# RoboSafe-Lab/Controllable-Latent-Diffusion-for-Traffic-Simulation

Measured on AMD Instinct MI355X. Metric: denoising-step·agent/s, higher is better.
Workload: dtype f32; 1 GPU; BASELINE configs[2]: 32 scenes x 64 agents per GPU, 100 denoising steps (DDPM ancestral loop of the reference), latent seq 52 x 4, cond 256, CFG w=2.0 (2 U-Net passes per step, non_cond_feat); target-speed guidance gradient through decoder + roll-out on every step t > 0; + LSTM decode + unicycle roll-out; scenes_total=32, agents_this_rank=2048, agents_total=2048, denoise_steps=100, guidance_gradient=True, sim_steps_per_bench_step=0, weights=random init (synth seed 0)

## Files before the change

controllable-latent-diffusion-for-traffic-simulation_amd/_lib.py:

```python
from __future__ import annotations

import ctypes as C
import os

PKG_DIR = os.path.dirname(os.path.abspath(__file__))
LIB_PATH = os.environ.get("CLD_LIB_PATH") or os.path.join(PKG_DIR, "libcld_hip.so")


class CldError(RuntimeError):
    pass


class CldConfig(C.Structure):
    _fields_ = [
        ("horizon", C.c_int32), ("latent_dim", C.c_int32), ("cond_dim", C.c_int32), ("base_dim", C.c_int32),
        ("dim_mults", C.c_int32 * 3), ("hidden", C.c_int32), ("n_timesteps", C.c_int32),
        ("step_time", C.c_float), ("acce_bound", C.c_float * 2), ("v_bound", C.c_float * 2),
        ("max_steer", C.c_float), ("max_yawvel", C.c_float),
        ("norm_mean", C.c_float * 6), ("norm_std", C.c_float * 6),
        ("precision", C.c_int32),
    ]


PRECISIONS = {"f32": 0, "f16x2": 1}
OPTIMIZERS = {"adam": 0, "sgd": 1}
KERNELS = {"guide": 0, "decode": 1, "encode": 2, "unet": 3, "context": 4, "conv5": 5}
KERNEL_FORMS = {
    "guide": {"auto": 0, "valu": 1, "mfma": 2, "quad": 3},
    "decode": {"auto": 0, "valu": 1, "mfma": 2},
    "encode": {"auto": 0, "valu": 1, "mfma": 2},
    "unet": {"auto": 0, "layers": 1, "chain": 2, "chain1": 3, "chain4": 4, "chainw": 5, "chainw2": 6, "chainw1": 7},
    "context": {"auto": 0, "direct": 1, "winograd": 2, "winograd_f2": 3},
    "conv5": {"auto": 0, "direct": 1, "winograd": 2, "winograd_whole": 3, "winograd_ksplit": 4},
}
FORMS = {name: v for forms in KERNEL_FORMS.values() for name, v in forms.items()}


def form_id(kind: str, name: str) -> int:
    if kind not in KERNEL_FORMS:
        raise ValueError(f"unknown kernel '{kind}' (one of {sorted(KERNEL_FORMS)})")
# ... 74 lines not shown
                                     C.c_int32, _P]),
    "cld_agent_collision": (C.c_int, [_P, _P, C.POINTER(CldCollision), _P, _P, _P, C.c_int32, _P]),
    "cld_map_collision_loss": (C.c_int, [_P, _P, C.POINTER(CldMapCollision), _P, _P, _P, C.c_int32, _P]),
    "cld_goal_loss": (C.c_int, [_P, _P, C.POINTER(CldGoal), _P, _P, _P, C.c_int32, _P]),
    "cld_set_goal_term": (C.c_int, [_P, C.POINTER(CldGoal)]),
    "cld_world_step": (C.c_int, [_P, _P, _P, _P, C.c_int32, _P, _P, C.c_int32, _P]),
    "cld_profile_enable": (C.c_int, [_P, C.c_int32]),
    "cld_profile_read": (C.c_int, [_P, C.POINTER(C.c_double), C.POINTER(C.c_int64), C.POINTER(C.c_double)]),
    "cld_profile_read_executed": (C.c_int, [_P, C.POINTER(C.c_double), C.POINTER(C.c_double), C.POINTER(C.c_double), C.POINTER(C.c_int32)]),
    "cld_set_stride": (C.c_int, [_P, C.c_int32]),
    "cld_debug_lds_floor": (C.c_int, [_P, C.c_size_t]),
    "cld_debug_force_kernel": (C.c_int, [_P, C.c_int32, C.c_int32]),
    "cld_debug_conv5_form": (C.c_int, [C.c_int32, C.c_int32, C.c_int32, C.c_int32, C.c_int64, C.c_int32]),
    "cld_debug_conv5_items": (C.c_int, [C.c_int32, C.c_int32, C.c_int64, C.c_int32]),
    "cld_debug_unet_span": (C.c_int, [_P, C.c_int32, _P, _P, _P, C.c_int32, _P, _P, C.c_int32, _P, C.c_size_t, _P]),
    "cld_debug_context_layer": (C.c_int, [_P, C.c_int32, _P, _P, _P, C.c_int32, C.c_int32, _P]),
    "cld_debug_context_pass_size": (C.c_int, [C.c_int32]),
    "cld_debug_stamps": (C.c_int, [_P, _P, C.c_int32]),
    "cld_debug_guide_stamps": (C.c_int, [_P]),
    "cld_unet_param_count": (C.c_int, [_P]),
    "cld_unet_param_info": (C.c_int, [_P, C.c_int32, C.POINTER(C.c_char_p), C.POINTER(C.c_size_t), C.POINTER(C.c_size_t),
                                      C.POINTER(C.c_int32), C.POINTER(C.c_int32)]),
    "cld_unet_param_floats": (C.c_size_t, [_P]),
    "cld_unet_tape_bytes": (C.c_size_t, [_P, C.c_int32]),
    "cld_unet_train_workspace_bytes": (C.c_size_t, [_P, C.c_int32]),
    "cld_unet_train_forward": (C.c_int, [_P, _P, _P, _P, _P, _P, _P, C.c_size_t, C.c_int32, _P, C.c_size_t, _P]),
    "cld_unet_backward": (C.c_int, [_P, _P, _P, _P, _P, _P, C.c_size_t, _P, _P, _P, _P, C.c_int32, C.c_int32, _P, C.c_size_t, _P]),
    "cld_vae_param_count": (C.c_int, [_P]),
    "cld_vae_param_info": (C.c_int, [_P, C.c_int32, C.POINTER(C.c_char_p), C.POINTER(C.c_size_t), C.POINTER(C.c_size_t),
                                     C.POINTER(C.c_int32), C.POINTER(C.c_int32)]),
# ... 36 lines not shown
```

controllable-latent-diffusion-for-traffic-simulation_amd/csrc/cld_api.hip:

```cpp
#include <hip/hip_runtime.h>

#include <cmath>
#include <cstdio>
#include <cstdlib>
#include <cstring>
#include <map>
#include <string>
#include <vector>

#include "../../include/cld.h"
#include "cld_kernels.h"
#include "train.h"

using namespace cld;

namespace {

constexpr int T = 52, D = 4, COND = 256, TE = 32, NCB = 1792, ACT = 3328;
constexpr int NBUF = 8;

struct ConvLayer {
    ConvGeom g{};
    bool has_a = false, has_b = false;
    float *wfrag = nullptr, *bias = nullptr, *gamma = nullptr, *beta = nullptr;
    float* ufrag_edge = nullptr;
    float* ufrag = nullptr;
    bool wino_launch = false;
    int c_out = 0, c1_real = 0, c1_pad = 0, c2 = 0, ly = 0, off0 = 0, orow0 = 0;
    int cb_off = -1;
};

struct ResBlock { ConvLayer c0, c1, res; bool has_res = false; };
constexpr long kProfStride = 10;
constexpr int kChainSmall = 944;
const char* const kResnet = "context_encoder.map_encoder.encoder_heads.map_model.";

}

struct cld_handle_s {
    cld_config cfg{};
    int stride = 1;
    int precision = CLD_PRECISION_F32;
// ... 21 lines not shown
    bool has_context = false;
    float *stem_w = nullptr, *stem_scale = nullptr, *stem_shift = nullptr;
    Conv2dLayer rn_conv[4][2][2], rn_ds[4];
    ContextHeadArgs ctx_head{};
    DynParams dyn{};
    bool prof_on = false;
    std::vector<hipEvent_t> prof_ev;
    size_t prof_used = 0;
    double prof_flop = 0.0;
    double prof_exec_flop = 0.0;
    double eval_alg_flop = 0.0, eval_exec_flop = 0.0;
    int eval_launches = 0;
    unsigned long long* stamp_buf = nullptr;
    int stamp_layer = -1, launch_counter = 0;
    size_t lds_floor = 0;
    long eval_counter = 0;
};

namespace {

int fail(cld_handle h, int code, const std::string& msg) {
    if (h) h->err = msg;
    return code;
}
#define HIPCK(h, expr)                                                                           \
    do {                                                                                         \
        hipError_t e__ = (expr);                                                                 \
        if (e__ != hipSuccess)                                                                   \
            return fail(h, CLD_ERR_HIP, std::string(#expr) + ": " + hipGetErrorString(e__));     \
    } while (0)
// ... 96 lines not shown
                        out[o++] = wget(16 * nt + (lane & 15), 16 * kgg + 4 * (lane >> 4) + s, t);
    return out;
}

template <class F>
std::vector<float> pack_latent_conv_weights(F&& wget, int c_out) {
    const int ntn = c_out / 16;
    std::vector<float> out((size_t)ntn * 64 * 8, 0.f);
    for (int nt = 0; nt < ntn; ++nt)
        for (int lane = 0; lane < 64; ++lane) {
            float* o = &out[((size_t)nt * 64 + lane) * 8];
            const int co = 16 * nt + (lane & 15), kk = lane >> 4;
            for (int s = 0; s < 4; ++s) o[s] = wget(co, s, kk);
            o[4] = wget(co, kk, 4);
        }
    return out;
}

constexpr float kWScale = 64.0f;
template <class F>
std::vector<float> pack_conv_weights_split(F&& wget, int c_out, int cin_virtual, int ntaps) {
    const int nchunk = cin_virtual / 32, ntn = c_out / 16;
    std::vector<_Float16> out((size_t)nchunk * ntaps * ntn * 1024);
    size_t o = 0;
    for (int c = 0; c < nchunk; ++c)
        for (int t = 0; t < ntaps; ++t)
            for (int nt = 0; nt < ntn; ++nt) {
                for (int plane = 0; plane < 2; ++plane)
                    for (int lane = 0; lane < 64; ++lane)
                        for (int j = 0; j < 8; ++j) {
// ... 128 lines not shown
    return conv5_takes_winograd(l.g.l_in, l.c1_real, l.c2, l.c_out, b_pad, h->force_kernel[CLD_KERNEL_CONV5]);
}
void count_flop(cld_handle h, const ConvLayer& l, int b_pad, double* alg, double* exec) {
    const double cin = (double)(l.c1_real + l.c2);
    *alg = 2.0 * (double)b_pad * l.g.lm * (l.g.ntaps * cin) * l.c_out;
    if (use_wino1d(h, l, b_pad)) *exec = 2.0 * (double)wino1d_row_planes(l.g.l_in, l.c_out, b_pad, wino_item_form(h)) * cin * l.c_out;
    else *exec = 2.0 * (double)b_pad * l.g.lm * (l.g.padc ? 20.0 : (double)(l.g.ntaps * (l.c1_pad + l.c2))) * l.c_out;
}
void count_launch(cld_handle h, const ConvLayer& l, int b_pad) {
    double alg, exec;
    count_flop(h, l, b_pad, &alg, &exec);
    h->eval_alg_flop += alg;
    h->eval_exec_flop += exec;
    h->eval_launches++;
}
hipError_t launch_one(cld_handle h, const ConvLayer& l, const ConvGeom& g, const ConvArgs& a, int b_pad, hipStream_t s) {
    count_launch(h, l, b_pad);
    if (use_wino1d(h, l, b_pad)) {
        ConvArgs w = a;
        w.wfrag = l.ufrag;
        w.wfrag_edge = l.ufrag_edge;
        return launch_wino1d(w, l.g.l_in, b_pad, wino_item_form(h), s);
    }
    return launch_conv(g, a, b_pad, s);
}
hipError_t launch_maybe_timed(cld_handle h, const ConvLayer& l, const ConvGeom& g, const ConvArgs& a, int b_pad, hipStream_t s) {
    const bool timed = h->prof_on && g.l_in == 13 && g.ntaps == 5 && g.epi == EPI_GN_MISH && l.c_out == 256 && l.c1_real == 256 &&
                       (h->eval_counter % kProfStride) == 0;
    if (!timed) return launch_one(h, l, g, a, b_pad, s);
    if (h->prof_used + 2 > h->prof_ev.size()) {
        for (int i = 0; i < 2; ++i) {
            hipEvent_t ev;
            hipError_t e = hipEventCreate(&ev);
            if (e != hipSuccess) return e;
            h->prof_ev.push_back(ev);
        }
    }
    hipError_t e = hipEventRecord(h->prof_ev[h->prof_used], s);
    if (e != hipSuccess) return e;
    e = launch_one(h, l, g, a, b_pad, s);
    if (e != hipSuccess) return e;
    e = hipEventRecord(h->prof_ev[h->prof_used + 1], s);
    h->prof_used += 2;
    double alg, exec;
    count_flop(h, l, b_pad, &alg, &exec);
    h->prof_flop += alg;
    h->prof_exec_flop += exec;
    return e;
}

hipError_t run_pair(cld_handle h, const ConvLayer& la, const ConvArgs& aa, const ConvLayer& lb, const ConvArgs& ab,
                    int b_pad, hipStream_t s) {
    ConvGeom ga, gb;
    if (!pick_tiling(la, b_pad, &ga, 2) || !pick_tiling(lb, b_pad, &gb, 2)) return hipErrorInvalidValue;
#ifdef CLD_EXPERIMENTS
// ... 3 lines not shown
    h->launch_counter += 2;
    if (use_wino1d(h, la, b_pad) || use_wino1d(h, lb, b_pad)) {
        hipError_t e = launch_maybe_timed(h, la, ga, aa, b_pad, s);
        return e != hipSuccess ? e : launch_maybe_timed(h, lb, gb, ab, b_pad, s);
    }
    if (ga.nwn == gb.nwn && ga.ks == gb.ks && conv_pair_supported(ga, gb)) {
        count_launch(h, la, b_pad);
        count_launch(h, lb, b_pad);
        h->eval_launches--;
        return launch_conv_pair(ga, aa, gb, ab, b_pad, s);
    }
    hipError_t e = launch_maybe_timed(h, la, ga, aa, b_pad, s);
    return e != hipSuccess ? e : launch_maybe_timed(h, lb, gb, ab, b_pad, s);
}

hipError_t run_args(cld_handle h, const ConvLayer& l, ConvArgs a, int b_pad, hipStream_t s);
hipError_t run_conv(cld_handle h, const ConvLayer& l, const float* x1, const float* x2, float* y, const float* res,
                    const float* cb, const float* tb_row, int b_pad, hipStream_t s) {
    return run_args(h, l, make_args(h, l, x1, x2, y, res, cb, tb_row), b_pad, s);
}
hipError_t run_args(cld_handle h, const ConvLayer& l, ConvArgs a, int b_pad, hipStream_t s) {
#ifdef CLD_EXPERIMENTS
    static const int stop_after = getenv("CLD_DEBUG_STOP") ? atoi(getenv("CLD_DEBUG_STOP")) : 1 << 30;
    if (h->launch_counter >= stop_after) return hipSuccess;
#endif
    a.stamps = (h->stamp_buf && h->launch_counter == h->stamp_layer) ? h->stamp_buf : nullptr;
    h->launch_counter++;
    ConvGeom g;
    if (!pick_tiling(l, b_pad, &g)) return hipErrorInvalidValue;
    return launch_maybe_timed(h, l, g, a, b_pad, s);
}

bool use_chains(cld_handle h, int b_pad) {
    if (h->precision != CLD_PRECISION_F32) return false;
    const int f = h->force_kernel[CLD_KERNEL_UNET];
    if (f == CLD_FORM_LAYERS) return false;
    if (f == CLD_FORM_CHAIN || f == CLD_FORM_CHAIN_TILE1 || f == CLD_FORM_CHAIN_TILE4 || f == CLD_FORM_CHAIN_WINO || f == CLD_FORM_CHAIN_WINO2 || f == CLD_FORM_CHAIN_WINO1) return true;
    (void)b_pad;
    return true;
}
int chain_tile(cld_handle h, int b_pad) {
    const int f = h->force_kernel[CLD_KERNEL_UNET];
    if (f == CLD_FORM_CHAIN_TILE1) return 1;
    if (f == CLD_FORM_CHAIN_TILE4 || f == CLD_FORM_CHAIN_WINO) return 4;
    return b_pad <= kChainSmall ? 1 : 4;
// ... 13 lines not shown
}

constexpr int kSpans = 12;
constexpr int kSpanIn[kSpans] = {-1, 6, 2, 4, 6, 2, 5, 2, 3, 2, 6, 3};
constexpr int kSpanSkip[kSpans] = {-1, -1, -1, -1, -1, -1, -1, -1, 5, -1, -1, 4};
constexpr int kSpanOut[kSpans] = {6, 2, 4, 6, 2, 5, 2, 3, 2, 6, 3, 7};
constexpr int kSpanL[kSpans + 1] = {52, 26, 26, 26, 13, 13, 13, 13, 13, 13, 13, 26, 52};
constexpr int kSpanC[kSpans + 1] = {4, 64, 128, 128, 128, 256, 256, 256, 256, 128, 128, 128, 4};
hipError_t run_unet_span(cld_handle h, const Ws& w, const float* x, int t_idx, int b_pad, int span, hipStream_t s) {
    const float* tbr = t_idx >= 0 ? h->tb + (size_t)t_idx * NCB : nullptr;
    float* const* b = w.buf;
    hipError_t e;
#define RC(...) do { e = run_conv(h, __VA_ARGS__, w.cb, tbr, b_pad, s); if (e != hipSuccess) return e; } while (0)
    auto resblock = [&](const ResBlock& rb, const float* in1, const float* in2, float* out) -> hipError_t {
        const float* r = in1;
        if (rb.has_res) {
            e = run_pair(h, rb.c0, make_args(h, rb.c0, in1, in2, b[1], nullptr, w.cb, tbr),
                         rb.res, make_args(h, rb.res, in1, in2, b[0], nullptr, w.cb, tbr), b_pad, s);
            if (e != hipSuccess) return e;
            r = b[0];
        } else {
            RC(rb.c0, in1, in2, b[1], nullptr);
        }
        RC(rb.c1, b[1], nullptr, out, r);
        return hipSuccess;
    };
#define RB(...) do { e = resblock(__VA_ARGS__); if (e != hipSuccess) return e; } while (0)
    switch (span) {
    case 0:
    if (use_chains(h, b_pad)) {
// ... 190 lines not shown
    return CLD_OK;
}

int cld_debug_lds_floor(cld_handle h, size_t bytes) {
    if (!h) return CLD_ERR_ARG;
    h->lds_floor = bytes;
    return CLD_OK;
}

int cld_debug_force_kernel(cld_handle h, int32_t which, int32_t form) {
    if (!h || which < 0 || which > 5 || form < 0 || form > (which == CLD_KERNEL_GUIDE || which == CLD_KERNEL_CONTEXT ? 3 : which == CLD_KERNEL_CONV5 ? 4 : (which == CLD_KERNEL_UNET ? 7 : 2))) return fail(h, CLD_ERR_ARG, "cld_debug_force_kernel: bad argument");
    h->force_kernel[which] = form;
    return CLD_OK;
}

int cld_debug_conv5_form(int32_t l_in, int32_t c1, int32_t c2, int32_t c_out, int64_t rows, int32_t forced_form) {
    if (l_in < 1 || c1 < 1 || c2 < 0 || c_out < 1 || rows < 0 || forced_form < 0 || forced_form > 4) return CLD_ERR_ARG;
    return conv5_takes_winograd(l_in, c1, c2, c_out, (long)((rows + 15) / 16 * 16), forced_form) ? CLD_FORM_WINOGRAD : CLD_FORM_DIRECT;
}

int cld_debug_conv5_items(int32_t l_in, int32_t c_out, int64_t rows, int32_t forced_form) {
    if ((l_in != 13 && l_in != 26) || (c_out != 64 && c_out != 128 && c_out != 256) || rows < 0 || rows > (1L << 30) || forced_form < 0 || forced_form > 4) return CLD_ERR_ARG;
    const int forced = forced_form == CLD_FORM_WINOGRAD_WHOLE ? 1 : forced_form == CLD_FORM_WINOGRAD_KSPLIT ? 2 : 0;
    return wino1d_item_form(l_in, c_out, (int)((rows + 15) / 16 * 16), forced);
}

int cld_profile_enable(cld_handle h, int32_t on) {
    if (!h) return CLD_ERR_ARG;
    h->prof_on = on != 0;
    h->prof_used = 0;
// ... 148 lines not shown
        const BlockDef& bd = kBlocks[i];
        ResBlock& rb = h->blocks[i];
        const std::string p = bd.name;
        const bool cat = (i == 8 || i == 10);
        const int c1 = cat ? bd.cin / 2 : bd.cin, c2 = cat ? bd.cin / 2 : 0;
        const bool latent_in = (i == 0);
        if ((rc = make_conv(rb.c0, p + ".blocks.0.block.0", bd.cout, c1, c2, bd.L, bd.L, 1, 5, k5, false, -2, 0, 1, bd.L,
                            EPI_GN_MISH, p + ".blocks.0.block.2", latent_in)) != CLD_OK) return rc;
        rb.c0.cb_off = cb_off;
        if ((rc = make_conv(rb.c1, p + ".blocks.1.block.0", bd.cout, bd.cout, 0, bd.L, bd.L, 1, 5, k5, false, -2, 0, 1,
                            bd.L, EPI_GN_MISH, p + ".blocks.1.block.2")) != CLD_OK) return rc;
        rb.has_res = bd.cin != bd.cout && !latent_in;
        if (rb.has_res)
            if ((rc = make_conv(rb.res, p + ".residual_conv", bd.cout, c1, c2, bd.L, bd.L, 1, 1, k1, false, 0, 0, 1, bd.L,
                                EPI_BIAS, "", latent_in)) != CLD_OK) return rc;
        if (latent_in) {
            UP(h->res4_w, *getw(h, p + ".residual_conv.weight"));
            UP(h->res4_b, *getw(h, p + ".residual_conv.bias"));
        }
        cb_off += bd.cout;
    }
    if ((rc = make_conv(h->down[0], "model.downs.0.2.conv", 64, 64, 0, 52, 26, 2, 3, k3, false, -1, 0, 1, 26, EPI_BIAS, ""))) return rc;
    if ((rc = make_conv(h->down[1], "model.downs.1.2.conv", 128, 128, 0, 26, 13, 2, 3, k3, false, -1, 0, 1, 13, EPI_BIAS, ""))) return rc;
    for (int u = 0; u < 2; ++u) {
        const std::string p = u == 0 ? "model.ups.0.2.conv" : "model.ups.1.2.conv";
        const int c = u == 0 ? 128 : 64, L = u == 0 ? 13 : 26;
        if ((rc = make_conv(h->upT[u][0], p, c, c, 0, L, L, 1, 2, kT_even, true, -1, 0, 2, 2 * L, EPI_BIAS, ""))) return rc;
        if ((rc = make_conv(h->upT[u][1], p, c, c, 0, L, L, 1, 2, kT_odd, true, 0, 1, 2, 2 * L, EPI_BIAS, ""))) return rc;
    }
    if ((rc = make_conv(h->final_cb, "model.final_conv.0.block.0", 64, 64, 0, 52, 52, 1, 5, k5, false, -2, 0, 1, 52,
// ... 1094 lines not shown
```

controllable-latent-diffusion-for-traffic-simulation_amd/csrc/cld_kernels.h:

```cpp
#pragma once
#include <hip/hip_runtime.h>
#include <stdint.h>

namespace cld {

inline hipError_t set_max_lds_once(const void* fn, int bytes, unsigned long long* done_mask) {
    int dev = 0;
    hipError_t e = hipGetDevice(&dev);
    if (e != hipSuccess) return e;
    if (dev >= 0 && dev < 64 && ((*done_mask >> dev) & 1ull)) return hipSuccess;
    e = hipFuncSetAttribute(fn, hipFuncAttributeMaxDynamicSharedMemorySize, bytes);
    if (e != hipSuccess) return e;
    if (dev >= 0 && dev < 64) *done_mask |= 1ull << dev;
    return hipSuccess;
}

constexpr int MT = 208;
constexpr int NMT = 13;

enum { EPI_BIAS = 0, EPI_GN_MISH = 1 };

struct ConvArgs {
    const float* x1;
    const float* x2;
// ... 34 lines not shown
    int gs;
    int ostr;
    int padc;
    int ain;
    int aout;
    int half;
};
hipError_t launch_conv(const ConvGeom& g, const ConvArgs& a, int b_pad, hipStream_t s);
bool conv_geom_supported(const ConvGeom& g);
hipError_t launch_conv_pair(const ConvGeom& ga, const ConvArgs& a, const ConvGeom& gb, const ConvArgs& b, int b_pad, hipStream_t s);
bool conv_pair_supported(const ConvGeom& a, const ConvGeom& b);
bool wino1d_supported(int l_in, int c1, int c2, int c_out);
hipError_t launch_wino1d(const ConvArgs& a, int l_in, int b_pad, int item_form, hipStream_t s);
int wino1d_item_form(int l_in, int c_out, int b_pad, int forced);
long wino1d_row_planes(int l_in, int c_out, int b_pad, int item_form);
hipError_t launch_wino1d_edge(const ConvArgs& a, int l_in, int b_pad, bool k_split, hipStream_t s);
long wino1d_edge_row_planes(int l_in, int b_pad);
long wino1d_gemm_rows(int l_in, int b_pad);
void set_lds_floor(size_t bytes);

enum { CHAIN_RES_NONE = 0, CHAIN_RES_LATENT = 1 ,
       CHAIN_RES_KEPT = 2 , CHAIN_RES_TENSOR = 3  };
struct ChainStage {
    const float* wfrag;
    const float* ufrag;
    const float* bias;
    const float* gamma;
    const float* beta;
    const float* res;
    int cb_off;
    int res_kind;
    int keep;
// ... 269 lines not shown
```

controllable-latent-diffusion-for-traffic-simulation_amd/csrc/wino1d_common.h:

```cpp
#pragma once
#include "cld_kernels.h"

namespace cld {

typedef float v4f __attribute__((ext_vector_type(4)));

#ifdef CLD_STAMPS
#define W1STAMP(k)                                                                                 \
    do {                                                                                           \
        __builtin_amdgcn_sched_barrier(0);                                                         \
        if (p.stamps && tid == 0) {                                                                \
            unsigned long long t_;                                                                 \
            asm volatile("s_memtime %0\n\ts_waitcnt lgkmcnt(0)" : "=s"(t_)::"memory");            \
            p.stamps[(size_t)blockIdx.x * 16 + (k)] = t_;                                          \
        }                                                                                          \
        __builtin_amdgcn_sched_barrier(0);                                                         \
    } while (0)
#define W1STAMP_RT(k)                                                                              \
    do {                                                                                           \
        if (p.stamps && tid == 0) {                                                                \
            unsigned long long t_;                                                                 \
            asm volatile("s_memrealtime %0\n\ts_waitcnt lgkmcnt(0)" : "=s"(t_)::"memory");        \
            p.stamps[(size_t)blockIdx.x * 16 + (k)] = t_;                                          \
        }                                                                                          \
// ... 35 lines not shown
    const v2f lo = mish2(v2f{x[0], x[1]}), hi = mish2(v2f{x[2], x[3]});
    return v4f{lo[0], lo[1], hi[0], hi[1]};
}

}

#define CLD_WINO1D_INSTANCES(X) \
    X(13, 256, 256, 256)        \
    X(13, 128, 128, 128)        \
    X(13, 128, 128, 256)        \
    X(13, 512, 256, 128)        \
    X(26, 128, 128, 128)        \
    X(26, 64, 64, 128)          \
    X(26, 256, 128, 64)

}
```

controllable-latent-diffusion-for-traffic-simulation_amd/csrc/wino1d_edge.hip:

```cpp
#include "wino1d_common.h"

#pragma clang fp contract(off)

namespace cld {

namespace {

template <int L_, int CIN_, int CS_, int COUT_>
struct E1Geo {
    static constexpr int L = L_, CIN = CIN_, CS = CS_, COUT = COUT_;
    static constexpr int AG = L == 13 ? 16 : 8;
    static constexpr int NT = L == 13 ? 3 : 4;
    static constexpr int NP = 8 + NT;
    static constexpr int NIT = 24 + NT;
    static constexpr int KC = 16, NCH = CIN / KC, NC1 = CS / KC, NCB = COUT / 64, NTN = COUT / 16;
    static constexpr int GS = COUT / 8;
    static constexpr int VB = 28 * 256;
    static constexpr int XCH = 2 * 4 * 16;
    static constexpr size_t LDS_BYTES = (2 * VB + XCH) * sizeof(float);
    static_assert(L == 13 || L == 26, "12 outputs by tiles + one direct column per row");
    static_assert(NCH % 2 == 0 && (CS == CIN || 2 * CS == CIN), "chunk pairs are unrolled; one source or two equal ones");
    static_assert(GS == 32 || GS == 16 || GS == 8, "a group is two waves' channels, one wave's or half of one's");
    static_assert(NCB == 1 || NCB == 2 || NCB == 4, "XCD-aware id mapping");
};

}

template <int L, int CIN, int CS, int COUT, int KS>
__global__ __launch_bounds__(256 * KS, KS == 1 ? 2 : 1) void wino1d_edge_kernel(const ConvArgs p, const int b_pad, const int xcd_map) {
    typedef E1Geo<L, CIN, CS, COUT> G;
    extern __shared__ __attribute__((aligned(16))) float lds1[];
    constexpr int VB = G::VB;
    float* xch = lds1 + 2 * KS * VB;
    const int tid = threadIdx.x, lane = tid & 63, i16 = lane & 15, kk = lane >> 4;
    const int wave8 = __builtin_amdgcn_readfirstlane(tid >> 6);
    const int wave = wave8 & 3, kh = KS == 1 ? 0 : wave8 >> 2;
    static_assert(KS == 1 || KS == 2, "one or two halves of the input channels");
    static_assert((G::NCH / KS) % 2 == 0, "chunk pairs are unrolled within a half");
    constexpr int NCK = G::NCH / KS;
    const int c_first = kh * NCK;
    int cb, grp;
    {
        const int e = blockIdx.x;
        if (xcd_map) {
            cb = (e >> 3) % G::NCB;
// ... 150 lines not shown
        const v4f p12 = acc[1][m] + acc[2][m], m12 = acc[1][m] - acc[2][m];
        const v4f p34 = acc[3][m] + acc[4][m], m34 = acc[3][m] - acc[4][m];
        const v4f p56 = acc[5][m] + acc[6][m], m56 = acc[5][m] - acc[6][m];
        Y[4 * m + 0] = ((acc[0][m] + p12) + (p34 + p56)) + bias;
        Y[4 * m + 1] = fma4(m56, 0.5f, fma4(m34, 2.0f, m12)) + bias;
        Y[4 * m + 2] = fma4(p56, 0.25f, fma4(p34, 4.0f, p12)) + bias;
        Y[4 * m + 3] = (fma4(m56, 0.125f, fma4(m34, 8.0f, m12)) + acc[7][m]) + bias;
    }
    Y[12] = accd + bias;
    __builtin_amdgcn_sched_barrier(0);
#pragma unroll
    for (int o = 0; o < 13; ++o) asm volatile("" : "+v"(Y[o]) : : "memory");
    const int ybytes = b_pad * L * COUT * 4;
    const __amdgpu_buffer_rsrc_t rsy = __builtin_amdgcn_make_buffer_rsrc(p.y, 0, ybytes, 0x00020000);
    const __amdgpu_buffer_rsrc_t rsr = __builtin_amdgcn_make_buffer_rsrc(const_cast<float*>(p.res ? p.res : p.y), 0, ybytes, 0x00020000);
    const bool has_res = p.res != nullptr;
    const int b = b0 + (L == 13 ? i16 : i16 >> 1), hh = L == 13 ? 0 : i16 & 1;
    const int obase = ((b * L + 12 * hh) * COUT + n4) * 4;
    const int odir = ((b * L + (L == 13 ? 12 : 24 + hh)) * COUT + n4) * 4;
    v4f rv[13];
    if (has_res) {
#pragma unroll
        for (int o = 0; o < 12; ++o) rv[o] = __builtin_bit_cast(v4f, __builtin_amdgcn_raw_buffer_load_b128(rsr, obase + o * (COUT * 4), 0, 0));
        rv[12] = __builtin_bit_cast(v4f, __builtin_amdgcn_raw_buffer_load_b128(rsr, odir, 0, 0));
    }
    v4f cbv = {0.f, 0.f, 0.f, 0.f};
    if (p.cbias) cbv = *reinterpret_cast<const v4f*>(p.cbias + (size_t)b * p.cb_stride + n4);
    const v4f gam = *reinterpret_cast<const v4f*>(p.gamma + n4), bet = *reinterpret_cast<const v4f*>(p.beta + n4);
    const v4f tb = p.tbias ? *reinterpret_cast<const v4f*>(p.tbias + n4) : v4f{0.f, 0.f, 0.f, 0.f};
    __builtin_amdgcn_sched_barrier(0);
    const float inv = 1.0f / (float)(G::GS * L);
    auto group_total = [&](float sv, float* scratch) {
        const auto r16 = __builtin_amdgcn_permlane16_swap(__builtin_bit_cast(unsigned, sv), __builtin_bit_cast(unsigned, sv), false, false);
        const unsigned a16 = r16[0], b16 = r16[1];
        sv = __builtin_bit_cast(float, a16) + __builtin_bit_cast(float, b16);
        if (G::GS >= 16) {
            const auto r32 = __builtin_amdgcn_permlane32_swap(__builtin_bit_cast(unsigned, sv), __builtin_bit_cast(unsigned, sv), false, false);
            const unsigned a32 = r32[0], b32 = r32[1];
            sv = __builtin_bit_cast(float, a32) + __builtin_bit_cast(float, b32);
// ... 20 lines not shown
        const v2f mm = {mean, mean};
        v2f q = {0.f, 0.f};
#pragma unroll
        for (int o = 0; o < 13; ++o) {
            const v2f d0 = lo2(Y[o]) - mm, d1 = hi2(Y[o]) - mm;
            q = __builtin_elementwise_fma(d0, d0, q);
            q = __builtin_elementwise_fma(d1, d1, q);
        }
        s2 = group_total(q[0] + q[1], xch + G::XCH / 2);
    }
    W1STAMP(3);
    {
        const v4f sc = (1.0f / sqrtf(s2 * inv + 1e-5f)) * gam;
        const v4f sh = __builtin_elementwise_fma(sc, v4f{-mean, -mean, -mean, -mean}, bet);
        const v4f add = tb + cbv;
#pragma unroll
        for (int o = 0; o < 13; ++o) {
            v4f v = mish4(__builtin_elementwise_fma(Y[o], sc, sh)) + add;
            if (has_res) v += rv[o];
            if (o < 12) __builtin_amdgcn_raw_buffer_store_b128(__builtin_bit_cast(u4v, v), rsy, obase + o * (COUT * 4), 0, 0);
            else __builtin_amdgcn_raw_buffer_store_b128(__builtin_bit_cast(u4v, v), rsy, odir, 0, 0);
        }
    }
    W1STAMP(4);
    W1STAMP_RT(9);
  } else if (PAIR) {
    __syncthreads();
    __syncthreads();
  }
}

long wino1d_edge_row_planes(int l_in, int b_pad) { return l_in == 13 ? 27L * b_pad : 56L * b_pad; }

template <int L, int CIN, int CS, int COUT>
static hipError_t launch_wino1d_edge_inst(const ConvArgs& a, int b_pad, bool k_split, hipStream_t s) {
    typedef E1Geo<L, CIN, CS, COUT> G;
    auto kern = wino1d_edge_kernel<L, CIN, CS, COUT, 1>;
    auto kern2 = wino1d_edge_kernel<L, CIN, CS, COUT, 2>;
    constexpr size_t lds2 = (4 * G::VB + G::XCH) * sizeof(float);
    static unsigned long long attr_done = 0, attr_done2 = 0;
    if (hipError_t e = set_max_lds_once(reinterpret_cast<const void*>(kern), (int)G::LDS_BYTES, &attr_done); e != hipSuccess) return e;
    if (hipError_t e = set_max_lds_once(reinterpret_cast<const void*>(kern2), (int)lds2, &attr_done2); e != hipSuccess) return e;
    if ((long)b_pad * L * CS * 4 >= (1L << 31) || (long)b_pad * L * COUT * 4 >= (1L << 31)) return hipErrorInvalidValue;
    const int groups = b_pad / G::AG;
    if (k_split) hipLaunchKernelGGL(kern2, dim3(groups * G::NCB), dim3(512), lds2, s, a, b_pad, groups % 8 == 0 ? 1 : 0);
    else hipLaunchKernelGGL(kern, dim3(groups * G::NCB), dim3(256), G::LDS_BYTES, s, a, b_pad, groups % 8 == 0 ? 1 : 0);
    return hipGetLastError();
}

hipError_t launch_wino1d_edge(const ConvArgs& a, int l_in, int b_pad, bool k_split, hipStream_t s) {
    if (b_pad < 16 || b_pad % 16 || a.res4_x || a.c1_real != a.c1_pad || (a.c2 != 0) != (a.x2 != nullptr)) return hipErrorInvalidValue;
#define X(L, CIN, CS, COUT) \
    if (l_in == L && a.c1_real == CS && a.c1_real + a.c2 == CIN && a.c_out == COUT) return launch_wino1d_edge_inst<L, CIN, CS, COUT>(a, b_pad, k_split, s);
    CLD_WINO1D_INSTANCES(X)
#undef X
    return hipErrorInvalidValue;
}

}
```

controllable-latent-diffusion-for-traffic-simulation_amd/engine.py:

```python
from __future__ import annotations

import contextlib
import ctypes as C
from typing import Mapping, Optional

import numpy as np
import torch

from . import _lib
from ._lib import CldConfig, CldError

T, D, COND = 52, 4, 256

CONTEXT_LAYERS = [(7, 2, 224, 34, 64)]
for _li in range(4):
    _c, _hin = 64 << _li, 56 >> max(_li - 1, 0)
    _s = 1 if _li == 0 else 2
    CONTEXT_LAYERS += [(3, _s, _hin, _c // _s, _c), (3, 1, _hin // _s, _c, _c), (3, 1, _hin // _s, _c, _c), (3, 1, _hin // _s, _c, _c)]
CONTEXT_LAYERS += [(1, 2, 56 >> (_li - 1), 32 << _li, 64 << _li) for _li in range(1, 4)]

UNET_SPANS = [(52, 4), (26, 64), (26, 128), (26, 128), (13, 128), (13, 256), (13, 256), (13, 256), (13, 256), (13, 128), (13, 128), (26, 128)]

def _ptr(t: Optional[torch.Tensor]):
    return None if t is None else C.c_void_p(t.data_ptr())
# ... 94 lines not shown
                self.lib.cld_destroy(self._h)
                self._h = None
        except Exception:
            pass

    def set_stride(self, stride: int):
        self._check(self.lib.cld_set_stride(self._h, int(stride)), "cld_set_stride")
        self.stride = int(stride)

    def force_kernel(self, which: str, form: str = "auto"):
        try:
            fid = _lib.form_id(which, form)
        except ValueError as ex:
            raise CldError(f"force_kernel: {ex}") from None
        self._check(self.lib.cld_debug_force_kernel(self._h, _lib.KERNELS[which], fid), "cld_debug_force_kernel")

    def debug_unet_span(self, span: int, x1, cond, t, x2=None):
        if not 0 <= span < len(UNET_SPANS):
            raise CldError(f"debug_unet_span: span {span} out of range")
        (L, C), (Lo, Co) = UNET_SPANS[span], (UNET_SPANS + [(52, 4)])[span + 1]
        B = int(x1.shape[0])
        x1 = self._f32(x1, (B, L, C))
        x2 = None if x2 is None else self._f32(x2, (B, L, C))
        cond = self._f32(cond, (B, 256))
        t_rows = None
        if isinstance(t, (int, np.integer)):
            t_idx = int(t)
        else:
            t_rows, t_idx = self._timesteps(t, B), 0
        y = torch.empty(B, Lo, Co, dtype=torch.float32, device=self.device)
# ... 680 lines not shown
```

include/cld.h:

```cpp
#ifndef CLD_H
#define CLD_H

#include <stddef.h>
#include <stdint.h>

#ifdef __cplusplus
extern "C" {
#endif

typedef struct cld_handle_s* cld_handle;

enum {
    CLD_OK = 0,
    CLD_ERR_ARG = -1,
    CLD_ERR_STATE = -2,
    CLD_ERR_WORKSPACE = -3,
    CLD_ERR_HIP = -4
};

typedef struct cld_config {
    int32_t horizon;
    int32_t latent_dim;
    int32_t cond_dim;
    int32_t base_dim;
// ... 176 lines not shown

int cld_compute_reward(cld_handle h, const float* traj, const float* traj_scaled, const float* raster_from_agent,
                       const uint8_t* drivable_map, int32_t H, int32_t W, const float* other_pos, const uint8_t* other_avail,
                       int32_t S, int32_t T_other, float collision_thresh, float* reward, float* offroad, float* collision,
                       int32_t B, void* stream);

int cld_guidance_losses(cld_handle h, const float* traj, const cld_guidance* guidance, float* losses, int32_t B, void* stream);

int cld_world_step(cld_handle h, const float* traj, const float* centroid, const float* yaw, int32_t k, float* world,
                   float* next_curr_states, int32_t B, void* stream);

int cld_debug_conv5_form(int32_t l_in, int32_t c1, int32_t c2, int32_t c_out, int64_t rows, int32_t forced_form);

int cld_debug_conv5_items(int32_t l_in, int32_t c_out, int64_t rows, int32_t forced_form);

int cld_debug_unet_span(cld_handle h, int32_t span, const float* x1, const float* x2, const float* cond, int32_t t_idx,
                        const int32_t* t_rows, float* y, int32_t B, void* workspace, size_t workspace_bytes, void* stream);

int cld_profile_enable(cld_handle h, int32_t on);
int cld_profile_read(cld_handle h, double* total_ms , int64_t* launches , double* total_flop );
int cld_profile_read_executed(cld_handle h, double* timed_executed_flop , double* eval_algorithmic_flop ,
                              double* eval_executed_flop , int32_t* eval_launches );

int cld_debug_stamps(cld_handle h, void* buf , int32_t layer);

int cld_debug_guide_stamps(void* out );

int cld_debug_lds_floor(cld_handle h, size_t bytes);

#define CLD_KERNEL_GUIDE 0
// ... 68 lines not shown
```

Before: 813,900 step·agent/s.

## Fold residual 1x1 projection into the second Winograd edge conv kernel

For resblocks with a residual 1x1 conv, the projection GEMM now runs inside the epilogue of the second conv's wino1d edge kernel. It stages the residual input chunks through LDS and accumulates them into the same MFMA output registers. This removes a separate residual launch and the write and read of the intermediate residual tensor. The cost is extra LDS traffic, register pressure and double-buffered syncs in the fused kernel, and it applies only to three instantiated shapes under f32 and item form 1.

```diff
diff --git a/controllable-latent-diffusion-for-traffic-simulation_amd/_lib.py b/controllable-latent-diffusion-for-traffic-simulation_amd/_lib.py
--- a/controllable-latent-diffusion-for-traffic-simulation_amd/_lib.py
+++ b/controllable-latent-diffusion-for-traffic-simulation_amd/_lib.py
@@ -24,6 +24,7 @@
 
 PRECISIONS = {"f32": 0, "f16x2": 1}
 OPTIMIZERS = {"adam": 0, "sgd": 1}
+RES_FOLD = {"fused": 0, "separate": 1}
 KERNELS = {"guide": 0, "decode": 1, "encode": 2, "unet": 3, "context": 4, "conv5": 5}
 KERNEL_FORMS = {
     "guide": {"auto": 0, "valu": 1, "mfma": 2, "quad": 3},
@@ -128,6 +129,8 @@
     "cld_debug_conv5_form": (C.c_int, [C.c_int32, C.c_int32, C.c_int32, C.c_int32, C.c_int64, C.c_int32]),
     "cld_debug_conv5_items": (C.c_int, [C.c_int32, C.c_int32, C.c_int64, C.c_int32]),
     "cld_debug_unet_span": (C.c_int, [_P, C.c_int32, _P, _P, _P, C.c_int32, _P, _P, C.c_int32, _P, C.c_size_t, _P]),
+    "cld_debug_res_fold": (C.c_int, [_P, C.c_int32]),
+    "cld_debug_pack_res_proj": (C.c_int64, [_P, C.c_int32, C.c_int32, _P, C.c_int64]),
     "cld_debug_context_layer": (C.c_int, [_P, C.c_int32, _P, _P, _P, C.c_int32, C.c_int32, _P]),
     "cld_debug_context_pass_size": (C.c_int, [C.c_int32]),
     "cld_debug_stamps": (C.c_int, [_P, _P, C.c_int32]),
diff --git a/controllable-latent-diffusion-for-traffic-simulation_amd/csrc/cld_api.hip b/controllable-latent-diffusion-for-traffic-simulation_amd/csrc/cld_api.hip
--- a/controllable-latent-diffusion-for-traffic-simulation_amd/csrc/cld_api.hip
+++ b/controllable-latent-diffusion-for-traffic-simulation_amd/csrc/cld_api.hip
@@ -26,6 +26,7 @@
     float* ufrag_edge = nullptr;
     float* ufrag = nullptr;
     bool wino_launch = false;
+    float* rfrag = nullptr;
     int c_out = 0, c1_real = 0, c1_pad = 0, c2 = 0, ly = 0, off0 = 0, orow0 = 0;
     int cb_off = -1;
 };
@@ -77,6 +78,7 @@
     unsigned long long* stamp_buf = nullptr;
     int stamp_layer = -1, launch_counter = 0;
     size_t lds_floor = 0;
+    int res_fold = CLD_RES_FOLD_FUSED;
     long eval_counter = 0;
 };
 
@@ -203,6 +205,12 @@
             for (int s = 0; s < 4; ++s) o[s] = wget(co, s, kk);
             o[4] = wget(co, kk, 4);
         }
+    return out;
+}
+
+std::vector<float> pack_res_proj(const float* W, int c_out, int c_in) {
+    std::vector<float> out = pack_conv_weights([&](int co, int ci, int) { return W[(size_t)co * c_in + ci]; }, c_out, c_in, 1);
+    out.resize((size_t)wino1d_edge_res_frag_floats(c_in, c_out), 0.f);
     return out;
 }
 
@@ -361,20 +369,24 @@
     h->eval_exec_flop += exec;
     h->eval_launches++;
 }
-hipError_t launch_one(cld_handle h, const ConvLayer& l, const ConvGeom& g, const ConvArgs& a, int b_pad, hipStream_t s) {
+hipError_t launch_one(cld_handle h, const ConvLayer& l, const ConvGeom& g, const ConvArgs& a, int b_pad, hipStream_t s, const ResProj* rp = nullptr) {
     count_launch(h, l, b_pad);
     if (use_wino1d(h, l, b_pad)) {
         ConvArgs w = a;
         w.wfrag = l.ufrag;
         w.wfrag_edge = l.ufrag_edge;
+        if (rp) {
+            w.wfrag = l.ufrag_edge;
+            return w.wfrag ? launch_wino1d_edge(w, l.g.l_in, b_pad, false, s, rp) : hipErrorInvalidValue;
+        }
         return launch_wino1d(w, l.g.l_in, b_pad, wino_item_form(h), s);
     }
-    return launch_conv(g, a, b_pad, s);
-}
-hipError_t launch_maybe_timed(cld_handle h, const ConvLayer& l, const ConvGeom& g, const ConvArgs& a, int b_pad, hipStream_t s) {
+    return rp ? hipErrorInvalidValue : launch_conv(g, a, b_pad, s);
+}
+hipError_t launch_maybe_timed(cld_handle h, const ConvLayer& l, const ConvGeom& g, const ConvArgs& a, int b_pad, hipStream_t s, const ResProj* rp = nullptr) {
     const bool timed = h->prof_on && g.l_in == 13 && g.ntaps == 5 && g.epi == EPI_GN_MISH && l.c_out == 256 && l.c1_real == 256 &&
                        (h->eval_counter % kProfStride) == 0;
-    if (!timed) return launch_one(h, l, g, a, b_pad, s);
+    if (!timed) return launch_one(h, l, g, a, b_pad, s, rp);
     if (h->prof_used + 2 > h->prof_ev.size()) {
         for (int i = 0; i < 2; ++i) {
             hipEvent_t ev;
@@ -385,7 +397,7 @@
     }
     hipError_t e = hipEventRecord(h->prof_ev[h->prof_used], s);
     if (e != hipSuccess) return e;
-    e = launch_one(h, l, g, a, b_pad, s);
+    e = launch_one(h, l, g, a, b_pad, s, rp);
     if (e != hipSuccess) return e;
     e = hipEventRecord(h->prof_ev[h->prof_used + 1], s);
     h->prof_used += 2;
@@ -419,12 +431,12 @@
     return e != hipSuccess ? e : launch_maybe_timed(h, lb, gb, ab, b_pad, s);
 }
 
-hipError_t run_args(cld_handle h, const ConvLayer& l, ConvArgs a, int b_pad, hipStream_t s);
+hipError_t run_args(cld_handle h, const ConvLayer& l, ConvArgs a, int b_pad, hipStream_t s, const ResProj* rp = nullptr);
 hipError_t run_conv(cld_handle h, const ConvLayer& l, const float* x1, const float* x2, float* y, const float* res,
                     const float* cb, const float* tb_row, int b_pad, hipStream_t s) {
     return run_args(h, l, make_args(h, l, x1, x2, y, res, cb, tb_row), b_pad, s);
 }
-hipError_t run_args(cld_handle h, const ConvLayer& l, ConvArgs a, int b_pad, hipStream_t s) {
+hipError_t run_args(cld_handle h, const ConvLayer& l, ConvArgs a, int b_pad, hipStream_t s, const ResProj* rp) {
 #ifdef CLD_EXPERIMENTS
     static const int stop_after = getenv("CLD_DEBUG_STOP") ? atoi(getenv("CLD_DEBUG_STOP")) : 1 << 30;
     if (h->launch_counter >= stop_after) return hipSuccess;
@@ -433,7 +445,14 @@
     h->launch_counter++;
     ConvGeom g;
     if (!pick_tiling(l, b_pad, &g)) return hipErrorInvalidValue;
-    return launch_maybe_timed(h, l, g, a, b_pad, s);
+    return launch_maybe_timed(h, l, g, a, b_pad, s, rp);
+}
+
+bool res_folds(cld_handle h, const ResBlock& rb, int b_pad) {
+    if (!rb.has_res || !rb.res.rfrag || h->precision != CLD_PRECISION_F32 || h->res_fold == CLD_RES_FOLD_SEPARATE) return false;
+    if (!use_wino1d(h, rb.c1, b_pad) || wino1d_item_form(rb.c1.g.l_in, rb.c1.c_out, b_pad, wino_item_form(h)) != 1) return false;
+    if ((long)b_pad * rb.c1.g.l_in * rb.res.c1_real * 4 >= (1L << 31)) return false;
+    return wino1d_edge_res_supported(rb.c1.g.l_in, rb.c1.c_out, rb.res.c1_real, rb.res.c2);
 }
 
 bool use_chains(cld_handle h, int b_pad) {
@@ -477,6 +496,14 @@
 #define RC(...) do { e = run_conv(h, __VA_ARGS__, w.cb, tbr, b_pad, s); if (e != hipSuccess) return e; } while (0)
     auto resblock = [&](const ResBlock& rb, const float* in1, const float* in2, float* out) -> hipError_t {
         const float* r = in1;
+        if (res_folds(h, rb, b_pad)) {
+            RC(rb.c0, in1, in2, b[1], nullptr);
+            const ResProj rp{in1, in2, rb.res.rfrag, rb.res.bias, rb.res.c1_real, rb.res.c2};
+            count_launch(h, rb.res, b_pad);
+            h->eval_launches--;
+            h->launch_counter++;
+            return run_args(h, rb.c1, make_args(h, rb.c1, b[1], nullptr, out, nullptr, w.cb, tbr), b_pad, s, &rp);
+        }
         if (rb.has_res) {
             e = run_pair(h, rb.c0, make_args(h, rb.c0, in1, in2, b[1], nullptr, w.cb, tbr),
                          rb.res, make_args(h, rb.res, in1, in2, b[0], nullptr, w.cb, tbr), b_pad, s);
@@ -697,6 +724,23 @@
     return CLD_OK;
 }
 
+int cld_debug_res_fold(cld_handle h, int32_t mode) {
+    if (!h || mode < CLD_RES_FOLD_FUSED || mode > CLD_RES_FOLD_SEPARATE) return fail(h, CLD_ERR_ARG, "cld_debug_res_fold: bad argument");
+    h->res_fold = mode;
+    return CLD_OK;
+}
+
+int64_t cld_debug_pack_res_proj(const float* w, int32_t c_out, int32_t c_in, float* out, int64_t capacity) {
+    if (c_out < 16 || c_out % 16 || c_in < 16 || c_in % 16) return CLD_ERR_ARG;
+    const int64_t n = wino1d_edge_res_frag_floats(c_in, c_out);
+    if (!w && !out) return n;
+    if (!w || !out || capacity < n) return CLD_ERR_ARG;
+    const std::vector<float> v = pack_res_proj(w, c_out, c_in);
+    if ((int64_t)v.size() != n) return CLD_ERR_STATE;
+    std::memcpy(out, v.data(), v.size() * sizeof(float));
+    return n;
+}
+
 int cld_debug_conv5_form(int32_t l_in, int32_t c1, int32_t c2, int32_t c_out, int64_t rows, int32_t forced_form) {
     if (l_in < 1 || c1 < 1 || c2 < 0 || c_out < 1 || rows < 0 || forced_form < 0 || forced_form > 4) return CLD_ERR_ARG;
     return conv5_takes_winograd(l_in, c1, c2, c_out, (long)((rows + 15) / 16 * 16), forced_form) ? CLD_FORM_WINOGRAD : CLD_FORM_DIRECT;
@@ -875,6 +919,8 @@
         if (rb.has_res)
             if ((rc = make_conv(rb.res, p + ".residual_conv", bd.cout, c1, c2, bd.L, bd.L, 1, 1, k1, false, 0, 0, 1, bd.L,
                                 EPI_BIAS, "", latent_in)) != CLD_OK) return rc;
+        if (rb.has_res && h->precision == CLD_PRECISION_F32 && wino1d_edge_res_supported(bd.L, bd.cout, c1, c2))
+            UP(rb.res.rfrag, pack_res_proj(getw(h, p + ".residual_conv.weight")->data(), bd.cout, c1 + c2));
         if (latent_in) {
             UP(h->res4_w, *getw(h, p + ".residual_conv.weight"));
             UP(h->res4_b, *getw(h, p + ".residual_conv.bias"));
diff --git a/controllable-latent-diffusion-for-traffic-simulation_amd/csrc/cld_kernels.h b/controllable-latent-diffusion-for-traffic-simulation_amd/csrc/cld_kernels.h
--- a/controllable-latent-diffusion-for-traffic-simulation_amd/csrc/cld_kernels.h
+++ b/controllable-latent-diffusion-for-traffic-simulation_amd/csrc/cld_kernels.h
@@ -72,8 +72,17 @@
 hipError_t launch_wino1d(const ConvArgs& a, int l_in, int b_pad, int item_form, hipStream_t s);
 int wino1d_item_form(int l_in, int c_out, int b_pad, int forced);
 long wino1d_row_planes(int l_in, int c_out, int b_pad, int item_form);
-hipError_t launch_wino1d_edge(const ConvArgs& a, int l_in, int b_pad, bool k_split, hipStream_t s);
+struct ResProj {
+    const float* x1;
+    const float* x2;
+    const float* wfrag;
+    const float* bias;
+    int c1, c2;
+};
+hipError_t launch_wino1d_edge(const ConvArgs& a, int l_in, int b_pad, bool k_split, hipStream_t s, const ResProj* rp = nullptr);
 long wino1d_edge_row_planes(int l_in, int b_pad);
+bool wino1d_edge_res_supported(int l_in, int c_out, int rc1, int rc2);
+long wino1d_edge_res_frag_floats(int c_in, int c_out);
 long wino1d_gemm_rows(int l_in, int b_pad);
 void set_lds_floor(size_t bytes);
 
diff --git a/controllable-latent-diffusion-for-traffic-simulation_amd/csrc/wino1d_common.h b/controllable-latent-diffusion-for-traffic-simulation_amd/csrc/wino1d_common.h
--- a/controllable-latent-diffusion-for-traffic-simulation_amd/csrc/wino1d_common.h
+++ b/controllable-latent-diffusion-for-traffic-simulation_amd/csrc/wino1d_common.h
@@ -73,4 +73,9 @@
     X(26, 64, 64, 128)          \
     X(26, 256, 128, 64)
 
+#define CLD_WINO1D_RES_INSTANCES(X) \
+    X(26, 128, 128, 128, 64, 64)    \
+    X(13, 256, 256, 256, 128, 128)  \
+    X(13, 128, 128, 128, 512, 256)
+
 }
diff --git a/controllable-latent-diffusion-for-traffic-simulation_amd/csrc/wino1d_edge.hip b/controllable-latent-diffusion-for-traffic-simulation_amd/csrc/wino1d_edge.hip
--- a/controllable-latent-diffusion-for-traffic-simulation_amd/csrc/wino1d_edge.hip
+++ b/controllable-latent-diffusion-for-traffic-simulation_amd/csrc/wino1d_edge.hip
@@ -1,3 +1,5 @@
+#include <type_traits>
+
 #include "wino1d_common.h"
 
 #pragma clang fp contract(off)
@@ -24,11 +26,51 @@
     static_assert(NCB == 1 || NCB == 2 || NCB == 4, "XCD-aware id mapping");
 };
 
-}
-
-template <int L, int CIN, int CS, int COUT, int KS>
-__global__ __launch_bounds__(256 * KS, KS == 1 ? 2 : 1) void wino1d_edge_kernel(const ConvArgs p, const int b_pad, const int xcd_map) {
+template <int L, int RCIN, int RCS, int NTN>
+struct ResStage {
+    static constexpr int RNCH = RCIN / 16, RNC1 = RCS / 16;
+    __amdgpu_buffer_rsrc_t rsq, rsq2, rsv;
+    int roff[4];
+    v4f q[4], rw, rbias;
+    __device__ __forceinline__ void init(const ResProj& rp, const int b_pad, const int b0, const int rr, const int cq, const int wave) {
+        const int rbytes = b_pad * L * RCS * 4;
+        rsq = __builtin_amdgcn_make_buffer_rsrc(const_cast<float*>(rp.x1), 0, rbytes, 0x00020000);
+        rsq2 = __builtin_amdgcn_make_buffer_rsrc(const_cast<float*>(RCS == RCIN ? rp.x1 : rp.x2), 0, rbytes, 0x00020000);
+        rsv = __builtin_amdgcn_make_buffer_rsrc(const_cast<float*>(rp.wfrag), 0, (RNCH + 1) * NTN * 1024, 0x00020000);
+        const int a = L == 13 ? rr : rr >> 1, h2 = L == 13 ? 0 : rr & 1;
+#pragma unroll
+        for (int g = 0; g < 4; ++g) {
+            const int o = wave + 4 * g;
+            const int pos = o < 12 ? 12 * h2 + o : (L == 13 ? 12 : 24 + h2);
+            roff[g] = o < 13 ? (((b0 + a) * L + pos) * RCS + 4 * cq) * 4 : rbytes;
+        }
+    }
+    __device__ __forceinline__ void load(const int c, const int wave) {
+#pragma unroll
+        for (int g = 0; g < 4; ++g) {
+            if (g == 3 && wave != 0) continue;
+            if (RCS == RCIN || c < RNC1) q[g] = __builtin_bit_cast(v4f, __builtin_amdgcn_raw_buffer_load_b128(rsq, roff[g], c * 64, 0));
+            else q[g] = __builtin_bit_cast(v4f, __builtin_amdgcn_raw_buffer_load_b128(rsq2, roff[g], (c - RNC1) * 64, 0));
+        }
+    }
+    __device__ __forceinline__ void store(float* img, const int wave) const {
+        float* vb = img + wave * 256;
+#pragma unroll
+        for (int g = 0; g < 4; ++g)
+            if (g < 3 || wave == 0) *reinterpret_cast<v4f*>(vb + g * 1024) = q[g];
+    }
+    __device__ __forceinline__ v4f wload(const int c, const int wvoff, const int wsoff) const {
+        return __builtin_bit_cast(v4f, __builtin_amdgcn_raw_buffer_load_b128(rsv, wvoff, c * (NTN * 1024) + wsoff, 0));
+    }
+};
+struct NoResStage {};
+
+}
+
+template <int L, int CIN, int CS, int COUT, int KS, int RCIN = 0, int RCS = 0>
+__global__ __launch_bounds__(256 * KS, KS == 1 ? 2 : 1) void wino1d_edge_kernel(const ConvArgs p, const int b_pad, const int xcd_map, const ResProj rp) {
     typedef E1Geo<L, CIN, CS, COUT> G;
+    static_assert(RCIN == 0 || (KS == 1 && RCIN % 32 == 0 && (RCS == RCIN || 2 * RCS == RCIN)), "the projection: four-wave items, chunk pairs, one source or two equal ones");
     extern __shared__ __attribute__((aligned(16))) float lds1[];
     constexpr int VB = G::VB;
     float* xch = lds1 + 2 * KS * VB;
@@ -209,7 +251,7 @@
     const int ybytes = b_pad * L * COUT * 4;
     const __amdgpu_buffer_rsrc_t rsy = __builtin_amdgcn_make_buffer_rsrc(p.y, 0, ybytes, 0x00020000);
     const __amdgpu_buffer_rsrc_t rsr = __builtin_amdgcn_make_buffer_rsrc(const_cast<float*>(p.res ? p.res : p.y), 0, ybytes, 0x00020000);
-    const bool has_res = p.res != nullptr;
+    const bool has_res = RCIN == 0 && p.res != nullptr;
     const int b = b0 + (L == 13 ? i16 : i16 >> 1), hh = L == 13 ? 0 : i16 & 1;
     const int obase = ((b * L + 12 * hh) * COUT + n4) * 4;
     const int odir = ((b * L + (L == 13 ? 12 : 24 + hh)) * COUT + n4) * 4;
@@ -218,6 +260,13 @@
 #pragma unroll
         for (int o = 0; o < 12; ++o) rv[o] = __builtin_bit_cast(v4f, __builtin_amdgcn_raw_buffer_load_b128(rsr, obase + o * (COUT * 4), 0, 0));
         rv[12] = __builtin_bit_cast(v4f, __builtin_amdgcn_raw_buffer_load_b128(rsr, odir, 0, 0));
+    }
+    [[maybe_unused]] std::conditional_t<(RCIN > 0), ResStage<L, RCIN, RCS, G::NTN>, NoResStage> rs;
+    if constexpr (RCIN > 0) {
+        rs.init(rp, b_pad, b0, rr, cq, wave);
+        rs.load(0, wave);
+        rs.rw = rs.wload(0, wvoff, wsoff);
+        rs.rbias = *reinterpret_cast<const v4f*>(rp.bias + n4);
     }
     v4f cbv = {0.f, 0.f, 0.f, 0.f};
     if (p.cbias) cbv = *reinterpret_cast<const v4f*>(p.cbias + (size_t)b * p.cb_stride + n4);
@@ -268,12 +317,51 @@
         const v4f sc = (1.0f / sqrtf(s2 * inv + 1e-5f)) * gam;
         const v4f sh = __builtin_elementwise_fma(sc, v4f{-mean, -mean, -mean, -mean}, bet);
         const v4f add = tb + cbv;
+        if constexpr (RCIN == 0) {
 #pragma unroll
         for (int o = 0; o < 13; ++o) {
             v4f v = mish4(__builtin_elementwise_fma(Y[o], sc, sh)) + add;
             if (has_res) v += rv[o];
             if (o < 12) __builtin_amdgcn_raw_buffer_store_b128(__builtin_bit_cast(u4v, v), rsy, obase + o * (COUT * 4), 0, 0);
             else __builtin_amdgcn_raw_buffer_store_b128(__builtin_bit_cast(u4v, v), rsy, odir, 0, 0);
+        }
+        } else {
+            constexpr int RNCH = RCIN / 16;
+            rs.store(lds1 + wofs, wave);
+#pragma unroll
+            for (int o = 0; o < 13; ++o) Y[o] = (mish4(__builtin_elementwise_fma(Y[o], sc, sh)) + add) + rs.rbias;
+            __syncthreads();
+            auto res_block = [&](const int buf, const int c, const bool stage) {
+                const v4f wcur = rs.rw;
+                rs.rw = rs.wload(c + 1, wvoff, wsoff);
+                if (stage) rs.load(c + 1, wave);
+                const int bo = buf * (VB * 4);
+                auto frag = [&](const int it) { return *reinterpret_cast<const v4f*>(ldsb + abase + bo + it * 1024); };
+                v4f ar[3];
+                ar[0] = frag(0);
+                ar[1] = frag(1);
+#pragma unroll
+                for (int o = 0; o < 13; ++o) {
+                    if (o + 2 < 13) ar[(o + 2) % 3] = frag(o + 2);
+                    __builtin_amdgcn_sched_barrier(0);
+#pragma unroll
+                    for (int e = 0; e < 4; ++e) Y[o] = __builtin_amdgcn_mfma_f32_16x16x4f32(wcur[e], ar[o % 3][e], Y[o], 0, 0, 0);
+                    __builtin_amdgcn_sched_barrier(0);
+                }
+                if (stage) rs.store(lds1 + (buf ^ 1) * VB + wofs, wave);
+            };
+#pragma clang loop unroll(disable)
+            for (int c = 0; c < RNCH; c += 2) {
+                res_block(0, c, true);
+                __syncthreads();
+                res_block(1, c + 1, c + 2 < RNCH);
+                __syncthreads();
+            }
+#pragma unroll
+            for (int o = 0; o < 13; ++o) {
+                if (o < 12) __builtin_amdgcn_raw_buffer_store_b128(__builtin_bit_cast(u4v, Y[o]), rsy, obase + o * (COUT * 4), 0, 0);
+                else __builtin_amdgcn_raw_buffer_store_b128(__builtin_bit_cast(u4v, Y[o]), rsy, odir, 0, 0);
+            }
         }
     }
     W1STAMP(4);
@@ -297,13 +385,44 @@
     if (hipError_t e = set_max_lds_once(reinterpret_cast<const void*>(kern2), (int)lds2, &attr_done2); e != hipSuccess) return e;
     if ((long)b_pad * L * CS * 4 >= (1L << 31) || (long)b_pad * L * COUT * 4 >= (1L << 31)) return hipErrorInvalidValue;
     const int groups = b_pad / G::AG;
-    if (k_split) hipLaunchKernelGGL(kern2, dim3(groups * G::NCB), dim3(512), lds2, s, a, b_pad, groups % 8 == 0 ? 1 : 0);
-    else hipLaunchKernelGGL(kern, dim3(groups * G::NCB), dim3(256), G::LDS_BYTES, s, a, b_pad, groups % 8 == 0 ? 1 : 0);
+    if (k_split) hipLaunchKernelGGL(kern2, dim3(groups * G::NCB), dim3(512), lds2, s, a, b_pad, groups % 8 == 0 ? 1 : 0, ResProj{});
+    else hipLaunchKernelGGL(kern, dim3(groups * G::NCB), dim3(256), G::LDS_BYTES, s, a, b_pad, groups % 8 == 0 ? 1 : 0, ResProj{});
     return hipGetLastError();
 }
 
-hipError_t launch_wino1d_edge(const ConvArgs& a, int l_in, int b_pad, bool k_split, hipStream_t s) {
+template <int L, int CIN, int CS, int COUT, int RCIN, int RCS>
+static hipError_t launch_wino1d_edge_res_inst(const ConvArgs& a, const ResProj& rp, int b_pad, hipStream_t s) {
+    typedef E1Geo<L, CIN, CS, COUT> G;
+    auto kern = wino1d_edge_kernel<L, CIN, CS, COUT, 1, RCIN, RCS>;
+    static unsigned long long attr_done = 0;
+    if (hipError_t e = set_max_lds_once(reinterpret_cast<const void*>(kern), (int)G::LDS_BYTES, &attr_done); e != hipSuccess) return e;
+    if ((long)b_pad * L * CS * 4 >= (1L << 31) || (long)b_pad * L * COUT * 4 >= (1L << 31) || (long)b_pad * L * RCS * 4 >= (1L << 31)) return hipErrorInvalidValue;
+    const int groups = b_pad / G::AG;
+    hipLaunchKernelGGL(kern, dim3(groups * G::NCB), dim3(256), G::LDS_BYTES, s, a, b_pad, groups % 8 == 0 ? 1 : 0, rp);
+    return hipGetLastError();
+}
+
+bool wino1d_edge_res_supported(int l_in, int c_out, int rc1, int rc2) {
+#define X(L, CIN, CS, COUT, RCIN, RCS) \
+    if (l_in == L && c_out == COUT && CIN == COUT && rc1 == RCS && rc1 + rc2 == RCIN) return true;
+    CLD_WINO1D_RES_INSTANCES(X)
+#undef X
+    return false;
+}
+
+long wino1d_edge_res_frag_floats(int c_in, int c_out) { return (long)(c_in / 16 + 1) * (c_out / 16) * 256; }
+
+hipError_t launch_wino1d_edge(const ConvArgs& a, int l_in, int b_pad, bool k_split, hipStream_t s, const ResProj* rp) {
     if (b_pad < 16 || b_pad % 16 || a.res4_x || a.c1_real != a.c1_pad || (a.c2 != 0) != (a.x2 != nullptr)) return hipErrorInvalidValue;
+    if (rp) {
+        if (k_split || a.res || !rp->x1 || !rp->wfrag || !rp->bias || (rp->c2 != 0) != (rp->x2 != nullptr)) return hipErrorInvalidValue;
+#define X(L, CIN, CS, COUT, RCIN, RCS) \
+        if (l_in == L && a.c1_real == CS && a.c1_real + a.c2 == CIN && a.c_out == COUT && rp->c1 == RCS && rp->c1 + rp->c2 == RCIN) \
+            return launch_wino1d_edge_res_inst<L, CIN, CS, COUT, RCIN, RCS>(a, *rp, b_pad, s);
+        CLD_WINO1D_RES_INSTANCES(X)
+#undef X
+        return hipErrorInvalidValue;
+    }
 #define X(L, CIN, CS, COUT) \
     if (l_in == L && a.c1_real == CS && a.c1_real + a.c2 == CIN && a.c_out == COUT) return launch_wino1d_edge_inst<L, CIN, CS, COUT>(a, b_pad, k_split, s);
     CLD_WINO1D_INSTANCES(X)
diff --git a/controllable-latent-diffusion-for-traffic-simulation_amd/engine.py b/controllable-latent-diffusion-for-traffic-simulation_amd/engine.py
--- a/controllable-latent-diffusion-for-traffic-simulation_amd/engine.py
+++ b/controllable-latent-diffusion-for-traffic-simulation_amd/engine.py
@@ -132,6 +132,11 @@
         except ValueError as ex:
             raise CldError(f"force_kernel: {ex}") from None
         self._check(self.lib.cld_debug_force_kernel(self._h, _lib.KERNELS[which], fid), "cld_debug_force_kernel")
+
+    def res_fold(self, mode: str = "fused"):
+        if mode not in _lib.RES_FOLD:
+            raise CldError(f"res_fold: unknown mode '{mode}' (one of {sorted(_lib.RES_FOLD)})")
+        self._check(self.lib.cld_debug_res_fold(self._h, _lib.RES_FOLD[mode]), "cld_debug_res_fold")
 
     def debug_unet_span(self, span: int, x1, cond, t, x2=None):
         if not 0 <= span < len(UNET_SPANS):
diff --git a/include/cld.h b/include/cld.h
--- a/include/cld.h
+++ b/include/cld.h
@@ -214,6 +214,12 @@
 
 int cld_debug_conv5_items(int32_t l_in, int32_t c_out, int64_t rows, int32_t forced_form);
 
+#define CLD_RES_FOLD_FUSED 0
+#define CLD_RES_FOLD_SEPARATE 1
+int cld_debug_res_fold(cld_handle h, int32_t mode);
+
+int64_t cld_debug_pack_res_proj(const float* w, int32_t c_out, int32_t c_in, float* out, int64_t capacity);
+
 int cld_debug_unet_span(cld_handle h, int32_t span, const float* x1, const float* x2, const float* cond, int32_t t_idx,
                         const int32_t* t_rows, float* y, int32_t B, void* workspace, size_t workspace_bytes, void* stream);
 
```

Measured after the change: 824,500 step·agent/s (median of 6 runs). +1.3%, better.
